# hkchengrex/Tracking-Anything-with-DEVA

Hardware: AMD Instinct MI355X
Metric: propagation FPS @480p (5 objects, working memory only) (higher is better)
Workload: dtype f32; 1 GPU; BASELINE configs[1]: DAVIS-2017-style 854x480 clip, 5 objects, working memory only (mem_every=5, top_k=30), recipe weights, one clip per GPU; parallelism=replicas x1

## Files before the change

tracking-anything-with-deva_amd/csrc/conv_wino.hip:

```cpp
#include <cstdlib>

#include "conv_args.h"

namespace deva {
namespace {

typedef float f32x16 __attribute__((ext_vector_type(16)));
typedef float f32x4 __attribute__((ext_vector_type(4)));
typedef float f32x2 __attribute__((ext_vector_type(2)));

__device__ __forceinline__ __amdgpu_buffer_rsrc_t make_rsrc(const void* base, int bytes) {
  return __builtin_amdgcn_make_buffer_rsrc(const_cast<void*>(base), 0, bytes, 0x00020000);
}
__device__ __forceinline__ f32x4 buf_load4(__amdgpu_buffer_rsrc_t r, int voff, int soff) {
  return __builtin_bit_cast(f32x4, __builtin_amdgcn_raw_buffer_load_b128(r, voff, soff, 0));
}

__device__ __forceinline__ f32x2 pk_add(f32x2 a, f32x2 b) {
  f32x2 r;
  asm("v_pk_add_f32 %0, %1, %2" : "=v"(r) : "v"(a), "v"(b));
  return r;
}
__device__ __forceinline__ f32x2 pk_sub(f32x2 a, f32x2 b) {
  f32x2 r;
  asm("v_pk_add_f32 %0, %1, %2 neg_lo:[0,1] neg_hi:[0,1]" : "=v"(r) : "v"(a), "v"(b));
  return r;
}

constexpr int WM = 64, WN = 64;
constexpr int KC = 8;
constexpr int TILE_FLOATS = 16 * 2 * 64 * 4;

struct WinoArgs {
  const float* in0;
  const float* in1;
  int64_t bs0, bs1;
  int c0, ctot;
  int H, W;
  int tiles_x, tiles_per_img, n_tiles;
  const float* u;
  const float* bias;
  int cout, cout_pad;
  int relu_in;
  const float* res;
  int64_t res_bs;
  int act;
  float* out;
  int blocks_m;
  int by_tiles;
};


template <bool RELU, bool RES>
__global__ __launch_bounds__(512, 1) void conv_wino_kernel(const WinoArgs p) {
  __shared__ __attribute__((aligned(16))) float sA[2][TILE_FLOATS];
  __shared__ __attribute__((aligned(16))) float sB[2][TILE_FLOATS];
  const int tid = threadIdx.x;
  const int lane = tid & 63;
  const int wave = __builtin_amdgcn_readfirstlane(tid >> 6);
  const int l31 = lane & 31, half = lane >> 5;
  const int wq = wave & 3, ph = wave >> 2;
  const int wm = wq >> 1, wn = wq & 1;
  int lb = blockIdx.x;
  if (p.by_tiles) {
    const int nb = gridDim.x, x = lb & 7, i = lb >> 3;
    lb = x * (nb >> 3) + min(x, nb & 7) + i;
  }
  const int block_m = lb % p.blocks_m, block_n = lb / p.blocks_m;
  const int m0 = block_m * WM, n0 = block_n * WN;

  const int c8 = wave, st = lane;
  const int sm = c8 >> 1, sh = c8 & 1;
  const int64_t HW = (int64_t)p.H * p.W;
  int poff[4];
  int poff_b0, poff_b1;
  bool lcol, rcol;
  {
    const int n = min(n0 + st, p.n_tiles - 1);
    const int b = n / p.tiles_per_img;
    const int r = n - b * p.tiles_per_img;
    const int ty = r / p.tiles_x, tx = r - ty * p.tiles_x;
    const int y0 = 2 * ty - 1, x0 = 2 * tx - 1;
    lcol = x0 >= 0;
    rcol = x0 + 3 < p.W;
#pragma unroll
    for (int i = 0; i < 4; ++i)
      poff[i] = (unsigned)(y0 + i) < (unsigned)p.H ? (int)(((int64_t)c8 * HW + (int64_t)(y0 + i) * p.W) * 4) : (int)0x80000000;
    poff_b0 = (int)(((int64_t)b * p.bs0 + x0) * 4);
    poff_b1 = (int)(((int64_t)b * p.bs1 + x0) * 4);
  }
  float pinf = __builtin_inff();
  asm("" : "+v"(pinf));
  const float llim = lcol ? __builtin_inff() : 0.0f, rlim = rcol ? __builtin_inff() : 0.0f;
  const int aoff = ((tid >> 6) * p.cout_pad + (tid & 63)) * 16;
  const int astride = 8 * p.cout_pad * 16;

  f32x16 acc[8];
#pragma unroll
  for (int q = 0; q < 8; ++q)
#pragma unroll
    for (int r = 0; r < 16; ++r) acc[q][r] = 0.0f;

  const int ksteps = p.ctot / KC;
  f32x4 ra[4], rb[4];
  auto load_step = [&](int s) {
    const float* ub = p.u + ((int64_t)s * 32 * p.cout_pad + m0) * 4;
    const __amdgpu_buffer_rsrc_t ru = make_rsrc(ub, 0x7fffffff);
#pragma unroll
    for (int i = 0; i < 4; ++i) ra[i] = buf_load4(ru, aoff, i * astride);
    const int c = s * KC;
    const bool first = c < p.c0;
    const float* base = (first ? p.in0 + (int64_t)c * HW : p.in1 + (int64_t)(c - p.c0) * HW) - 4;
    const __amdgpu_buffer_rsrc_t rx = make_rsrc(base, 0x7fffffff);
    const int pb = (first ? poff_b0 : poff_b1) + 16;
#pragma unroll
    for (int i = 0; i < 4; ++i) rb[i] = buf_load4(rx, pb + poff[i], 0);
  };
  auto store_step = [&](int buf) {
    float* a = sA[buf];
#pragma unroll
    for (int i = 0; i < 4; ++i) *reinterpret_cast<f32x4*>(a + (tid + 512 * i) * 4) = ra[i];
    float* bdst = sB[buf] + (sh * 4 + sm) * 64 + st;
    f32x2 dl[4], dr[4];
#pragma unroll
    for (int i = 0; i < 4; ++i) {
      const f32x4 v = rb[i];
      if (RELU) {
        dl[i] = f32x2{__builtin_amdgcn_fmed3f(v[0], 0.0f, llim), __builtin_amdgcn_fmed3f(v[1], 0.0f, pinf)};
        dr[i] = f32x2{__builtin_amdgcn_fmed3f(v[2], 0.0f, pinf), __builtin_amdgcn_fmed3f(v[3], 0.0f, rlim)};
      } else {
        dl[i] = f32x2{lcol ? v[0] : 0.0f, v[1]};
        dr[i] = f32x2{v[2], rcol ? v[3] : 0.0f};
      }
    }
    f32x2 wl[4], wr[4];
    wl[0] = pk_sub(dl[0], dl[2]);
    wl[1] = pk_add(dl[1], dl[2]);
    wl[2] = pk_sub(dl[2], dl[1]);
    wl[3] = pk_sub(dl[1], dl[3]);
    wr[0] = pk_sub(dr[0], dr[2]);
    wr[1] = pk_add(dr[1], dr[2]);
    wr[2] = pk_sub(dr[2], dr[1]);
    wr[3] = pk_sub(dr[1], dr[3]);
#pragma unroll
    for (int i = 0; i < 4; ++i) {
      f32x2 lo, hi;
      asm("v_pk_add_f32 %0, %1, %2 op_sel:[0,0] op_sel_hi:[1,0] neg_lo:[0,1]" : "=v"(lo) : "v"(wl[i]), "v"(wr[i]));
      asm("v_pk_add_f32 %0, %1, %2 op_sel:[0,1] op_sel_hi:[1,1] neg_lo:[0,1] neg_hi:[1,0]" : "=v"(hi) : "v"(wr[i]), "v"(wl[i]));
      bdst[(4 * i + 0) * 8 * 64] = lo[0];
      bdst[(4 * i + 1) * 8 * 64] = lo[1];
      bdst[(4 * i + 2) * 8 * 64] = hi[0];
      bdst[(4 * i + 3) * 8 * 64] = hi[1];
    }
  };

  f32x4 fa[2][2], fb[2][2];
  auto read_frag = [&](int buf, int set, int g) {
    const float* a_rd = sA[buf] + ((8 * ph) * 2 * 64 + half * 64 + wm * 32 + l31) * 4;
    const float* b_rd = sB[buf] + ((8 * ph) * 2 + half) * 4 * 64 + wn * 32 + l31;
#pragma unroll
    for (int j = 0; j < 2; ++j) {
      const int q = 2 * g + j;
      fa[set][j] = *reinterpret_cast<const f32x4*>(a_rd + q * 2 * 64 * 4);
#pragma unroll
      for (int e = 0; e < 4; ++e) fb[set][j][e] = b_rd[(q * 2 * 4 + e) * 64];
    }
  };
  auto multiply = [&](int set, int g) {
#pragma unroll
    for (int e = 0; e < 4; ++e)
#pragma unroll
      for (int j = 0; j < 2; ++j)
        acc[2 * g + j] = __builtin_amdgcn_mfma_f32_32x32x2f32(fa[set][j][e], fb[set][j][e], acc[2 * g + j], 0, 0, 0);
  };
  load_step(0);
  store_step(0);
  __syncthreads();
  read_frag(0, 0, 0);
  for (int s = 0; s < ksteps; ++s) {
    const int buf = s & 1;
    const bool more = s + 1 < ksteps;
    if (more) load_step(s + 1);
#pragma unroll
    for (int g = 0; g < 3; ++g) {
      read_frag(buf, (g + 1) & 1, g + 1);
      multiply(g & 1, g);
      if (RELU && g == 2 && more) store_step(buf ^ 1);
    }
    if (!RELU && more) store_step(buf ^ 1);
    __syncthreads();
    if (more) read_frag(buf ^ 1, 0, 0);
    multiply(1, 3);
  }

  float* xch = sA[0] + (wq * 16 * 4) * 64 + lane;
  const int n = n0 + wn * 32 + l31;
  const bool n_ok = n < p.n_tiles;
  if (ph == 1) {
#pragma unroll
    for (int r = 0; r < 16; ++r) {
      float y[2][2];
      {
        const float a0 = acc[0][r], a1 = acc[1][r], a2 = acc[2][r], a3 = acc[3][r];
        y[0][0] = a0 + a1 + a2;
        y[0][1] = a1 - a2 - a3;
        const float b0 = -acc[0][r] - acc[4][r], b1 = -acc[1][r] - acc[5][r], b2 = -acc[2][r] - acc[6][r], b3 = -acc[3][r] - acc[7][r];
        y[1][0] = b0 + b1 + b2;
        y[1][1] = b1 - b2 - b3;
      }
#pragma unroll
      for (int a = 0; a < 2; ++a)
#pragma unroll
        for (int j = 0; j < 2; ++j) xch[(r * 4 + a * 2 + j) * 64] = y[a][j];
    }
  }
  __syncthreads();
  if (ph == 1 || !n_ok) return;
  int64_t o_base;
  int r_off;
  bool row1;
  {
    const int b = n / p.tiles_per_img;
    const int rr = n - b * p.tiles_per_img;
    const int ty = rr / p.tiles_x, tx = rr - ty * p.tiles_x;
    const int64_t pix = (int64_t)(2 * ty) * p.W + 2 * tx;
    o_base = (int64_t)b * p.cout * HW + pix;
    r_off = (int)(((int64_t)b * p.res_bs + pix) * 4);
    row1 = 2 * ty + 1 < p.H;
  }
  const __amdgpu_buffer_rsrc_t rres = make_rsrc(RES ? p.res : p.out, RES ? 0x7fffffff : 0);
#pragma unroll
  for (int rh = 0; rh < 2; ++rh) {
    f32x2 rv[8][2];
    float bv[8];
#pragma unroll
    for (int k = 0; k < 8; ++k) {
      const int r = rh * 8 + k;
      const int m = m0 + wm * 32 + (r & 3) + 8 * (r >> 2) + 4 * half;
      bv[k] = p.bias ? p.bias[min(m, p.cout - 1)] : 0.0f;
      if (RES) {
        const int mo = m < p.cout ? r_off + (int)((int64_t)m * HW * 4) : (int)0x80000000;
#pragma unroll
        for (int a = 0; a < 2; ++a)
          rv[k][a] = __builtin_bit_cast(f32x2, __builtin_amdgcn_raw_buffer_load_b64(rres, (a == 0 || row1) ? mo + a * p.W * 4 : (int)0x80000000, 0, 0));
      } else {
        rv[k][0] = rv[k][1] = f32x2{0.0f, 0.0f};
      }
    }
    __builtin_amdgcn_sched_barrier(0);
#pragma unroll
    for (int k = 0; k < 8; ++k) {
      const int r = rh * 8 + k;
      const int m = m0 + wm * 32 + (r & 3) + 8 * (r >> 2) + 4 * half;
      if (m >= p.cout) continue;
      float y[2][2];
      {
        const float a0 = acc[0][r] + acc[4][r], a1 = acc[1][r] + acc[5][r], a2 = acc[2][r] + acc[6][r], a3 = acc[3][r] + acc[7][r];
        y[0][0] = a0 + a1 + a2;
        y[0][1] = a1 - a2 - a3;
        const float b0 = acc[4][r], b1 = acc[5][r], b2 = acc[6][r], b3 = acc[7][r];
        y[1][0] = b0 + b1 + b2;
        y[1][1] = b1 - b2 - b3;
      }
      const int64_t o = o_base + (int64_t)m * HW;
#pragma unroll
      for (int a = 0; a < 2; ++a) {
        f32x2 v;
#pragma unroll
        for (int j = 0; j < 2; ++j) {
          float x = (y[a][j] + xch[(r * 4 + a * 2 + j) * 64]) + bv[k] + rv[k][a][j];
          if (p.act == DEVA_ACT_RELU) {
            x = fmaxf(x, 0.0f);
          } else if (p.act == DEVA_ACT_SIGMOID) {
            x = sigmoidf_(x);
          } else if (p.act == DEVA_ACT_SQUARE_PLUS_ONE) {
            x = x * x + 1.0f;
          }
          v[j] = x;
        }
        if (a == 0 || row1) *reinterpret_cast<f32x2*>(p.out + o + (int64_t)a * p.W) = v;
      }
    }
    __builtin_amdgcn_sched_barrier(0);
  }
}

}

int launch_conv_wino(const ConvArgs& a, const float* u, hipStream_t st) {
  if (!u || !a.vec_ok || a.KH != 3 || a.KW != 3 || a.stride != 1 || a.pad != 1 || (a.W & 1) || a.W < 4) return -1;
  if (a.c0 % KC || a.ctot % KC || a.cout < 32) return -1;
  if (a.in0_span >= (1ll << 29) || a.in1_span >= (1ll << 29)) return -1;
  if (a.res && (int64_t)(a.n_total / a.OHW) * a.res_bs >= (1ll << 29)) return -1;
  WinoArgs p;
  p.in0 = a.in0;
  p.in1 = a.in1 ? a.in1 : a.in0;
  p.bs0 = a.bs0;
  p.bs1 = a.bs1;
  p.c0 = a.c0;
  p.ctot = a.ctot;
  p.H = a.H;
  p.W = a.W;
  p.tiles_x = a.W / 2;
  p.tiles_per_img = ((a.H + 1) / 2) * (a.W / 2);
  const int batch = a.n_total / a.OHW;
  p.n_tiles = batch * p.tiles_per_img;
  p.u = u;
  p.bias = a.bias;
  p.cout = a.cout;
  p.cout_pad = (a.cout + 63) / 64 * 64;
  p.relu_in = a.relu_in;
  p.res = a.res;
  p.res_bs = a.res_bs;
  p.act = a.act;
  p.out = a.out;
  p.blocks_m = p.cout_pad / WM;
  p.by_tiles = (int64_t)batch * a.HW > 16ll * p.cout_pad;
#if defined(DEVA_CONV_PROBES) || defined(DEVA_WINO_TUNE)
  static const int min_blocks_probe = [] {
    const char* e = getenv("DEVA_WINO_MIN_BLOCKS");
    return e ? atoi(e) : 160;
  }();
  const int min_blocks = min_blocks_probe;
  static const int by_tiles_probe = [] {
    const char* e = getenv("DEVA_WINO_BY_TILES");
    return e ? atoi(e) : -1;
  }();
  if (by_tiles_probe >= 0) p.by_tiles = by_tiles_probe;
#else
  const int min_blocks = 160;
#endif
  const int64_t blocks = (int64_t)p.blocks_m * ceil_div(p.n_tiles, WN);
  if (blocks < min_blocks) return -1;
  const dim3 grid((unsigned)blocks), block(512);
  if (p.relu_in) {
    if (p.res) {
      hipLaunchKernelGGL((conv_wino_kernel<true, true>), grid, block, 0, st, p);
    } else {
      hipLaunchKernelGGL((conv_wino_kernel<true, false>), grid, block, 0, st, p);
    }
  } else {
    if (p.res) {
      hipLaunchKernelGGL((conv_wino_kernel<false, true>), grid, block, 0, st, p);
    } else {
      hipLaunchKernelGGL((conv_wino_kernel<false, false>), grid, block, 0, st, p);
    }
  }
  return check_launch("deva_conv2d (Winograd F(2x2, 3x3))");
}

}

extern "C" int64_t deva_conv_pack_wino(const float* w_oihw, float* out, int cout, int cin) {
  using namespace deva;
  if (!w_oihw || cout <= 0 || cin <= 0) {
    set_error("deva_conv_pack_wino: bad arguments");
    return -1;
  }
  if (cin % 8) return -1;
  const int cout_pad = (cout + 63) / 64 * 64;
  const int64_t elems = (int64_t)(cin / 8) * 16 * 2 * cout_pad * 4;
  if (!out) return elems;
  for (int64_t i = 0; i < elems; ++i) out[i] = 0.0f;
  static const double G[4][3] = {{1.0, 0.0, 0.0}, {0.5, 0.5, 0.5}, {0.5, -0.5, 0.5}, {0.0, 0.0, 1.0}};
  for (int m = 0; m < cout; ++m)
    for (int c = 0; c < cin; ++c) {
      const float* g = w_oihw + ((int64_t)m * cin + c) * 9;
      double t[4][3];
      for (int i = 0; i < 4; ++i)
        for (int j = 0; j < 3; ++j) t[i][j] = G[i][0] * g[0 * 3 + j] + G[i][1] * g[1 * 3 + j] + G[i][2] * g[2 * 3 + j];
      for (int i = 0; i < 4; ++i)
        for (int l = 0; l < 4; ++l) {
          const double u = t[i][0] * G[l][0] + t[i][1] * G[l][1] + t[i][2] * G[l][2];
          const int q = 4 * i + l;
          out[((((int64_t)(c / 8) * 16 + q) * 2 + (c & 1)) * cout_pad + m) * 4 + (c % 8) / 2] = (float)u;
        }
    }
  return elems;
}
```

Before: 158.0 frames/s.

## Load Winograd weights directly to LDS and deepen the K-loop pipeline

Transformed weight tiles now go straight from global memory into shared memory through buffer-load-to-LDS, instead of passing through registers and a separate store. The K loop is restructured into a two-step unrolled pipeline that prefetches activations and weights two steps ahead. It uses compile-time buffer indices and a custom barrier that waits with vmcnt(4), so loads in flight can overlap the barrier. Probe-only ablation switches are added. The aim is less register pressure and VGPR round-trips, and better hiding of global latency, at the risk of subtle wait-count or LDS hazard bugs.

```diff
diff --git a/tracking-anything-with-deva_amd/csrc/conv_wino.hip b/tracking-anything-with-deva_amd/csrc/conv_wino.hip
--- a/tracking-anything-with-deva_amd/csrc/conv_wino.hip
+++ b/tracking-anything-with-deva_amd/csrc/conv_wino.hip
@@ -1,4 +1,5 @@
 #include <cstdlib>
+#include <type_traits>
 
 #include "conv_args.h"
 
@@ -27,9 +28,19 @@
   return r;
 }
 
+#ifdef DEVA_CONV_PROBES
+#define WINO_ABL(bit) (p.ablate & (bit))
+#else
+#define WINO_ABL(bit) false
+#endif
+
 constexpr int WM = 64, WN = 64;
 constexpr int KC = 8;
 constexpr int TILE_FLOATS = 16 * 2 * 64 * 4;
+
+template <int N>
+__device__ __forceinline__ constexpr std::integral_constant<int, (N ^ 1)> flip_buf(std::integral_constant<int, N>) { return {}; }
+__device__ __forceinline__ int flip_buf(int b) { return b ^ 1; }
 
 struct WinoArgs {
   const float* in0;
@@ -48,13 +59,15 @@
   float* out;
   int blocks_m;
   int by_tiles;
+  int ablate;
 };
 
 
 template <bool RELU, bool RES>
 __global__ __launch_bounds__(512, 1) void conv_wino_kernel(const WinoArgs p) {
-  __shared__ __attribute__((aligned(16))) float sA[2][TILE_FLOATS];
-  __shared__ __attribute__((aligned(16))) float sB[2][TILE_FLOATS];
+  __shared__ __attribute__((aligned(16))) float smem[4 * TILE_FLOATS];
+#define sA(b) (smem + (b) * TILE_FLOATS)
+#define sB(b) (smem + (2 + (b)) * TILE_FLOATS)
   const int tid = threadIdx.x;
   const int lane = tid & 63;
   const int wave = __builtin_amdgcn_readfirstlane(tid >> 6);
@@ -102,12 +115,19 @@
     for (int r = 0; r < 16; ++r) acc[q][r] = 0.0f;
 
   const int ksteps = p.ctot / KC;
-  f32x4 ra[4], rb[4];
-  auto load_step = [&](int s) {
+  f32x4 rb[4];
+  auto load_w = [&](int s, auto bufc) {
+    const int buf = bufc;
+    if (WINO_ABL(8)) return;
     const float* ub = p.u + ((int64_t)s * 32 * p.cout_pad + m0) * 4;
     const __amdgpu_buffer_rsrc_t ru = make_rsrc(ub, 0x7fffffff);
 #pragma unroll
-    for (int i = 0; i < 4; ++i) ra[i] = buf_load4(ru, aoff, i * astride);
+    for (int i = 0; i < 4; ++i)
+      __builtin_amdgcn_raw_ptr_buffer_load_lds(ru, (__attribute__((address_space(3))) void*)(sA(buf) + (wave * 64 + 512 * i) * 4), 16, aoff,
+                                               i * astride, 0, 0);
+  };
+  auto load_act = [&](int s) {
+    if (WINO_ABL(2)) return;
     const int c = s * KC;
     const bool first = c < p.c0;
     const float* base = (first ? p.in0 + (int64_t)c * HW : p.in1 + (int64_t)(c - p.c0) * HW) - 4;
@@ -116,11 +136,9 @@
 #pragma unroll
     for (int i = 0; i < 4; ++i) rb[i] = buf_load4(rx, pb + poff[i], 0);
   };
-  auto store_step = [&](int buf) {
-    float* a = sA[buf];
-#pragma unroll
-    for (int i = 0; i < 4; ++i) *reinterpret_cast<f32x4*>(a + (tid + 512 * i) * 4) = ra[i];
-    float* bdst = sB[buf] + (sh * 4 + sm) * 64 + st;
+  auto stage_act = [&](auto bufc) {
+    const int buf = bufc;
+    float* bdst = sB(buf) + (sh * 4 + sm) * 64 + st;
     f32x2 dl[4], dr[4];
 #pragma unroll
     for (int i = 0; i < 4; ++i) {
@@ -147,6 +165,10 @@
       f32x2 lo, hi;
       asm("v_pk_add_f32 %0, %1, %2 op_sel:[0,0] op_sel_hi:[1,0] neg_lo:[0,1]" : "=v"(lo) : "v"(wl[i]), "v"(wr[i]));
       asm("v_pk_add_f32 %0, %1, %2 op_sel:[0,1] op_sel_hi:[1,1] neg_lo:[0,1] neg_hi:[1,0]" : "=v"(hi) : "v"(wr[i]), "v"(wl[i]));
+      if (WINO_ABL(1)) {
+        asm volatile("" ::"v"(lo), "v"(hi));
+        continue;
+      }
       bdst[(4 * i + 0) * 8 * 64] = lo[0];
       bdst[(4 * i + 1) * 8 * 64] = lo[1];
       bdst[(4 * i + 2) * 8 * 64] = hi[0];
@@ -155,9 +177,12 @@
   };
 
   f32x4 fa[2][2], fb[2][2];
-  auto read_frag = [&](int buf, int set, int g) {
-    const float* a_rd = sA[buf] + ((8 * ph) * 2 * 64 + half * 64 + wm * 32 + l31) * 4;
-    const float* b_rd = sB[buf] + ((8 * ph) * 2 + half) * 4 * 64 + wn * 32 + l31;
+  const float* a_rd0 = sA(0) + ((8 * ph) * 2 * 64 + half * 64 + wm * 32 + l31) * 4;
+  const float* b_rd0 = sB(0) + ((8 * ph) * 2 + half) * 4 * 64 + wn * 32 + l31;
+  auto read_frag = [&](auto bufc, int set, int g) {
+    const int buf = bufc;
+    const float* a_rd = a_rd0 + buf * TILE_FLOATS;
+    const float* b_rd = b_rd0 + buf * TILE_FLOATS;
 #pragma unroll
     for (int j = 0; j < 2; ++j) {
       const int q = 2 * g + j;
@@ -173,27 +198,55 @@
       for (int j = 0; j < 2; ++j)
         acc[2 * g + j] = __builtin_amdgcn_mfma_f32_32x32x2f32(fa[set][j][e], fb[set][j][e], acc[2 * g + j], 0, 0, 0);
   };
-  load_step(0);
-  store_step(0);
-  __syncthreads();
-  read_frag(0, 0, 0);
-  for (int s = 0; s < ksteps; ++s) {
-    const int buf = s & 1;
-    const bool more = s + 1 < ksteps;
-    if (more) load_step(s + 1);
+  auto wg_barrier = [&]() {
+    if (WINO_ABL(4)) return;
+    asm volatile("s_waitcnt vmcnt(4) lgkmcnt(0)\n\ts_barrier" ::: "memory");
+  };
+  constexpr std::integral_constant<int, 0> B0{};
+  constexpr std::integral_constant<int, 1> B1{};
+
+  auto step = [&](auto bufc, int s) {
+    const auto other = flip_buf(bufc);
+    const bool tile1 = s == 0 && ksteps > 1;
+    auto stage_tile1 = [&]() {
+      stage_act(other);
+      load_act(min(2, ksteps - 1));
+    };
 #pragma unroll
     for (int g = 0; g < 3; ++g) {
-      read_frag(buf, (g + 1) & 1, g + 1);
+      read_frag(bufc, (g + 1) & 1, g + 1);
       multiply(g & 1, g);
-      if (RELU && g == 2 && more) store_step(buf ^ 1);
-    }
-    if (!RELU && more) store_step(buf ^ 1);
-    __syncthreads();
-    if (more) read_frag(buf ^ 1, 0, 0);
+      if (RELU && g == 2 && tile1) stage_tile1();
+    }
+    if (!RELU && tile1) stage_tile1();
+    wg_barrier();
+    if (s + 1 < ksteps) read_frag(other, 0, 0);
+    if (s + 2 < ksteps) {
+      stage_act(bufc);
+      load_w(s + 2, bufc);
+      load_act(min(s + 3, ksteps - 1));
+    }
     multiply(1, 3);
-  }
-
-  float* xch = sA[0] + (wq * 16 * 4) * 64 + lane;
+  };
+
+  load_act(0);
+  load_w(0, B0);
+  stage_act(B0);
+  asm volatile("s_waitcnt vmcnt(0) lgkmcnt(0)\n\ts_barrier" ::: "memory");
+  read_frag(B0, 0, 0);
+  if (ksteps > 1) {
+    load_w(1, B1);
+    load_act(1);
+  }
+  for (int s = 0;;) {
+    step(B0, s);
+    if (++s == ksteps) break;
+    step(B1, s);
+    if (++s == ksteps) break;
+  }
+  asm volatile("s_waitcnt vmcnt(0)" ::: "memory");
+
+  float* xch = sA(0) + (wq * 16 * 4) * 64 + lane;
   const int n = n0 + wn * 32 + l31;
   const bool n_ok = n < p.n_tiles;
   if (ph == 1) {
@@ -284,6 +337,9 @@
     __builtin_amdgcn_sched_barrier(0);
   }
 }
+
+#undef sA
+#undef sB
 
 }
 
@@ -315,6 +371,14 @@
   p.act = a.act;
   p.out = a.out;
   p.blocks_m = p.cout_pad / WM;
+  p.ablate = 0;
+#ifdef DEVA_CONV_PROBES
+  static const int ablate_probe = [] {
+    const char* e = getenv("DEVA_WINO_ABLATE");
+    return e ? atoi(e) : 0;
+  }();
+  p.ablate = ablate_probe;
+#endif
   p.by_tiles = (int64_t)batch * a.HW > 16ll * p.cout_pad;
 #if defined(DEVA_CONV_PROBES) || defined(DEVA_WINO_TUNE)
   static const int min_blocks_probe = [] {
```

Result: faster. 162.8 frames/s, median of 6 (+3.1%).
